# quokka-astro/quokka

Hardware: AMD Instinct MI355X
Metric: Mcell-updates/s on 3D Sedov unigrid (higher is better)
Workload: dtype f64; 1 GPU; 3D Sedov blast 256x256x256 unigrid (tests/blast_unigrid_256.in scaled to 256^3 cells per GPU), 128^3 boxes, PPM+HLLC RK2, gamma=1.4, CFL 0.3, reflecting octant; cells_per_gpu=16777216, boxes_per_gpu=8, parallelism=box-decomposition x1, rk2_mode=carry, fofc_stages=0, retries=0, x_sweep_in_y_march=True

## Files before the change

### include/quokka_amd.h

```cpp
#ifndef QUOKKA_AMD_H_
#define QUOKKA_AMD_H_

#include <stdint.h>

#ifdef __cplusplus
extern "C" {
#endif

typedef struct qk_ctx qk_ctx;
typedef struct qk_level qk_level;
typedef void *qk_stream;

typedef enum qk_status {
	QK_OK = 0,
	QK_ERR_INVALID = -1,
	QK_ERR_HIP = -2,
	QK_ERR_UNSUPPORTED = -3,
	QK_ERR_STATE = -4,
	QK_ERR_NOT_CONVERGED = -5
} qk_status;

typedef struct qk_array4 {
	double *p;
	int64_t jstride, kstride, nstride;
// ... 95 lines not shown
typedef struct qk_hydro_stage_args {
	const qk_array4 *U_in;
	const qk_array4 *U_old;
	qk_array4 *U_out;
	qk_array4 *halfFlux[3];
	qk_array4 *halfVel[3];
	qk_iarray4 *redoFlag;
	int64_t *d_redo_count;
	int *d_error_flag;
	double *d_max_signal;
	void *scratch;
	int64_t scratch_bytes;
	double dx[3];
	double dt;
	int stage;
	int reconstruction_order;
	double densityFloor, tempFloor;
	int use_dual_energy;
	double K_visc;
	int store_flux_rk2;
	qk_array4 *fluxRk2[3];
	int rk2_carry_rhs;
	qk_array4 *rhs1;
	const struct qk_carray4 *flux_mask;
	int fofc_pass;
	int prim_out;
	int prim_in;
	int store_vel_rk2;
	qk_array4 *velRk2[3];
} qk_hydro_stage_args;

int64_t qk_hydro_stage_scratch_bytes(qk_level *lev, const qk_hydro_traits *t);
int qk_hydro_stage_fused(qk_level *lev, qk_stream s, const qk_hydro_traits *t, const qk_hydro_stage_args *a);

#define QK_MAX_GROUPS 8
typedef struct qk_rad_traits {
	double c_light, c_hat, radiation_constant, Erad_floor;
	int beta_order;
	int opacity_model;
	double kappaP, kappaE, kappaF;
	int pow_mode;
	int eddington_model;
	double opacity_T_ref, opacity_T_exponent, opacity_pow_floor;
	int ngroups;
	int mg_opacity_model;
	double energy_unit;
	double rad_boundaries[QK_MAX_GROUPS + 1];
	double mg_kappa_exponent[QK_MAX_GROUPS + 1], mg_kappa_lower[QK_MAX_GROUPS + 1];
	double mg_kappa_rho_exponent, mg_kappa_T_ref, mg_kappa_T_exponent;
	int enable_dust_gas_thermal_coupling_model;
	double dust_gas_interaction_coeff;
	int thermal_model;
	double gas_dust_coupling_threshold;
	double cooling_linear_coeff[QK_MAX_GROUPS];
	double cr_heating_rate;
	int enable_photoelectric_heating;
	double pe_heating_E1_derivative;
} qk_rad_traits;

int qk_rad_ConservedToPrimitive(qk_level *lev, qk_stream s, const qk_rad_traits *rt, const qk_array4 *cons, qk_array4 *primVar, int nghost);
int qk_rad_ComputeWavespeedCorrection(qk_level *lev, qk_stream s, const qk_rad_traits *rt, const qk_hydro_traits *t, int ndim, const qk_array4 *consVar,
				      const double dx[3], qk_array4 *const eps[3]);
int qk_rad_ComputeFluxes(qk_level *lev, qk_stream s, const qk_rad_traits *rt, int dir, qk_array4 *x1Flux, const qk_array4 *x1LeftState,
			 const qk_array4 *x1RightState, const qk_array4 *consVar, const qk_array4 *wavespeed_eps);
int qk_rad_computeRadiationFluxes(qk_level *lev, qk_stream s, const qk_rad_traits *rt, int ndim, int reconstruction_order, const qk_array4 *consVar,
				  qk_array4 *const flux[3], const qk_array4 *const wavespeed_eps[3] );
// ... 200 lines not shown
```

### quokka_amd/capi.py

```python
from __future__ import annotations

import ctypes as C
import os

_HERE = os.path.dirname(os.path.abspath(__file__))
LIB_PATH = os.environ.get("QK_LIB_PATH", os.path.join(_HERE, "lib", "libquokka_amd.so"))

QK_OK, QK_ERR_INVALID, QK_ERR_HIP, QK_ERR_UNSUPPORTED, QK_ERR_STATE, QK_ERR_NOT_CONVERGED = 0, -1, -2, -3, -4, -5
ERR_UNSUPPORTED = QK_ERR_UNSUPPORTED
QK_TRACER_PREV, QK_TRACER_CUR, QK_TRACER_MAX_DEPTH = 0, 1, 3
HOOK_COMPILED = 100
DIR_X1, DIR_X2, DIR_X3 = 0, 1, 2
ARITH_DIVBY_RECIPOF, ARITH_DIVN, ARITH_RECIPEXACT, ARITH_SQRTN = 0, 1, 2, 3
COOLING_LIBM_DEVICE, COOLING_LIBM_PORTABLE = 0, 1
RIEMANN_HLLC, RIEMANN_LLF, RIEMANN_HLLD = 0, 1, 2
LIMITER_MINMOD, LIMITER_MC = 0, 1
BC_REFLECT_ODD, BC_INT_DIR, BC_REFLECT_EVEN, BC_FOEXTRAP, BC_EXT_DIR = -1, 0, 1, 2, 3

K_B = 1.380649e-16
M_U = 1.6605390666e-24


class Array4(C.Structure):
    _fields_ = [("p", C.c_void_p), ("jstride", C.c_int64), ("kstride", C.c_int64), ("nstride", C.c_int64),
# ... 118 lines not shown
    L.qk_ReconstructStatesConstant.argtypes = [vp, vp, ci, vp, vp, vp, ci, ci]
    L.qk_ReconstructStatesPLM.argtypes = [vp, vp, ci, ci, vp, vp, vp, ci, ci]
    L.qk_ReconstructStatesPPM.argtypes = [vp, vp, ci, vp, vp, vp, ci, ci, ci, ci]
    L.qk_hydro_ConservedToPrimitive.argtypes = [vp, vp, T, vp, vp, ci]
    L.qk_hydro_ComputeFlatteningCoefficients.argtypes = [vp, vp, T, ci, vp, vp, ci]
    L.qk_hydro_FlattenShocks.argtypes = [vp, vp, T, ci, vp, vp, vp, vp, vp, vp, ci, ci]
    L.qk_hydro_ComputeFluxes.argtypes = [vp, vp, T, ci, ci, vp, vp, vp, vp, vp, cd]
    L.qk_hydro_ComputeRhsFromFluxes.argtypes = [vp, vp, T, vp, P(vp), P(cd), ci]
    L.qk_hydro_AddInternalEnergyPdV.argtypes = [vp, vp, T, vp, vp, P(cd), P(vp), vp]
    L.qk_hydro_PredictStep.argtypes = [vp, vp, T, vp, vp, vp, cd, ci, vp, vp]
    L.qk_hydro_EnforceLimits.argtypes = [vp, vp, T, cd, cd, vp]
    L.qk_hydro_SyncDualEnergy.argtypes = [vp, vp, T, vp, vp]
    L.qk_hydro_ComputeMaxSignalSpeed.argtypes = [vp, vp, T, vp, vp]
    L.qk_hydro_maxSignalSpeedLocal.argtypes = [vp, vp, T, ci, vp, vp]
    L.qk_replaceFluxes.argtypes = [vp, vp, ci, vp, vp, vp, ci]
    L.qk_Saxpy.argtypes = [vp, vp, ci, vp, cd, vp, ci]
    R = P(RadTraits)
    L.qk_rad_ConservedToPrimitive.argtypes = [vp, vp, R, vp, vp, ci]
    L.qk_rad_ComputeFluxes.argtypes = [vp, vp, R, ci, vp, vp, vp, vp, vp]
    L.qk_rad_computeRadiationFluxes.argtypes = [vp, vp, R, ci, ci, vp, P(vp), P(vp)]
    L.qk_rad_ComputeWavespeedCorrection.argtypes = [vp, vp, R, T, ci, vp, P(cd), P(vp)]
    L.qk_rad_PredictStep.argtypes = [vp, vp, R, ci, vp, vp, P(vp), cd, P(cd)]
    L.qk_rad_AddFluxesRK2.argtypes = [vp, vp, R, ci, vp, vp, vp, P(vp), P(vp), cd, P(cd)]
    L.qk_hydro_FixupState.argtypes = [vp, vp, T, cd, cd, ci, vp, vp, vp]
    L.qk_rad_stage_fused.argtypes = [vp, vp, R, ci, ci, vp, vp, vp, vp, P(vp), cd, P(cd), P(vp)]
    L.qk_rad_AddSourceTermsSingleGroup.argtypes = [vp, vp, R, T, vp, vp, cd, ci, vp, vp]
    L.qk_rad_AddSourceTermsSingleGroupMirror.argtypes = [vp, vp, R, T, vp, vp, cd, ci, vp, vp, vp]
    L.qk_rad_AddSourceTermsMultiGroup.argtypes = [vp, vp, R, T, vp, vp, cd, ci, vp, vp]
    L.qk_rad_mg_planck_fractions.argtypes = [vp, R, cd, ci, P(cd), P(cd), P(cd)]
    if hasattr(L, "qk_hydro_stage_fused"):
        L.qk_hydro_stage_scratch_bytes.argtypes = [vp, T]
        L.qk_hydro_stage_scratch_bytes.restype = C.c_int64
        L.qk_hydro_stage_fused.argtypes = [vp, vp, T, P(StageArgs)]
    if hasattr(L, "qk_ghost_plan_create"):
        L.qk_ghost_plan_create.argtypes = [vp, P(vp), P(Geometry), ci, ci, ci, P(Box), P(ci), ci]
        L.qk_ghost_plan_destroy.argtypes = [vp]
        L.qk_ghost_plan_num_peers.argtypes = [vp]
        L.qk_ghost_plan_peer.argtypes = [vp, ci, P(ci), P(C.c_int64), P(C.c_int64)]
        L.qk_ghost_plan_num_items.argtypes = [vp, ci, ci]
        L.qk_ghost_plan_item.argtypes = [vp, ci, ci, ci, P(ci), P(ci), ci * 3, ci * 3, ci * 3, P(C.c_int64)]
        L.qk_FillBoundary_local.argtypes = [vp, vp, vp]
        L.qk_FillBoundary_local_int.argtypes = [vp, vp, vp]
        L.qk_FillBoundary_pack.argtypes = [vp, vp, ci, vp, vp]
        L.qk_FillBoundary_unpack.argtypes = [vp, vp, ci, vp, vp]
        L.qk_SumBoundary_local.argtypes = [vp, vp, vp]
        L.qk_SumBoundary_pack.argtypes = [vp, vp, ci, vp, vp]
        L.qk_SumBoundary_unpack.argtypes = [vp, vp, ci, vp, vp]
        L.qk_FillBoundary_pack_int.argtypes = [vp, vp, ci, vp, vp]
        L.qk_FillBoundary_unpack_int.argtypes = [vp, vp, ci, vp, vp]
        L.qk_FillPhysicalBoundary.argtypes = [vp, vp, vp, P(BCRec), P(DirichletFace)]
        L.qk_FillPhysicalBoundary_subset.argtypes = [vp, vp, vp, P(BCRec), P(DirichletFace), C.c_int]
        L.qk_ghost_plan_set_components.argtypes = [vp, C.c_int, C.c_int]
        L.qk_ghost_plan_box_is_remote.argtypes = [vp, C.c_int]
        L.qk_ghost_plan_set_box_remote.argtypes = [vp, C.c_int, C.c_int]
    if hasattr(L, "qk_tag_relative_gradient"):
        L.qk_tag_relative_gradient.argtypes = [vp, vp, T, vp, vp, ci, C.c_double, C.c_double, ci]
        L.qk_tag_centered_gradient.argtypes = [vp, vp, vp, vp, ci, ci, C.c_double, C.c_double, C.c_double, ci]
        L.qk_avgdown_plan_create.argtypes = [vp, vp, ci * 3, P(vp)]
        L.qk_avgdown_plan_destroy.argtypes = [vp]
        L.qk_avgdown_plan_num_items.argtypes = [vp]
        L.qk_average_down.argtypes = [vp, vp, vp, vp, ci, ci]
        L.qk_interp_plan_create.argtypes = [vp, vp, P(Geometry), ci, ci * 3, ci, ci, vp, P(vp)]
        L.qk_interp_plan_destroy.argtypes = [vp]
        L.qk_interp_plan_num_items.argtypes = [vp]
        L.qk_interp_plan_item.argtypes = [vp, ci, P(ci), P(ci), ci * 3, ci * 3]
        L.qk_InterpFromCoarse.argtypes = [vp, vp, vp, vp, vp, C.c_double, C.c_double, ci, ci, ci]
# ... 32 lines not shown
    L.qk_tracer_AdvectWithUmac.argtypes = [vp, vp, vp * 3, cd, C.c_int64, vp * 3, vp * 3]
    L.qk_tracer_Redistribute.argtypes = [vp, vp, C.c_int64, vp * 3, vp]
    L.qk_tracer_plan_create_refined.argtypes = [vp, P(vp), P(Geometry), cd * 3, cd * 3, cd * 3]
    L.qk_tracer_plan_set_parent.argtypes = [vp, ci, vp, vp * 3]
    L.qk_tracer_plan_set_time_weights.argtypes = [vp, cd, cd]
    L.qk_tracer_plan_clear_parent.argtypes = [vp]
    L.qk_tracer_Where.argtypes = [P(vp), ci, vp, ci, ci, C.c_int64, vp * 3, vp, vp, vp]
    i3 = ci * 3
    L.qk_gravity_scratch_bytes.argtypes = [i3]
    L.qk_gravity_scratch_bytes.restype = C.c_int64
    L.qk_gravity_num_ghosts.argtypes = [i3]
    L.qk_gravity_num_ghosts.restype = C.c_int64
    L.qk_gravity_fill_rhs.argtypes = [vp, vp, cd, vp, ci, i3, vp]
    L.qk_gravity_dirichlet_solve.argtypes = [vp, vp, i3, cd, vp, vp, cd, cd, ci, vp, C.c_int64, P(ci), P(cd)]
    L.qk_gravity_surface_gather.argtypes = [vp, vp, i3, vp, vp]
    L.qk_gravity_surface_potential.argtypes = [vp, vp, i3, vp, vp, vp, C.c_int64]
    L.qk_gravity_surface_scatter.argtypes = [vp, vp, i3, vp, vp]
    L.qk_gravity_kick.argtypes = [vp, vp, i3, vp, cd * 3, cd, vp]
    _lib = L
    return L


BOXES_ALL, BOXES_LOCAL_ONLY, BOXES_REMOTE_DEPENDENT = 0, 1, 2
TAG_CLEAR, TAG_BUF, TAG_SET = 0, 1, 2
TAGFIELD_PRESSURE = -1

DECLARED_SYMBOLS = [
    "qk_ctx_create", "qk_ctx_destroy", "qk_last_error", "qk_version", "qk_level_create", "qk_level_destroy",
    "qk_upload_array4_table", "qk_upload_iarray4_table", "qk_clear_bytes", "qk_profile_enable", "qk_profile_only", "qk_profile_reset", "qk_profile_num_kernels", "qk_profile_get",
    "qk_ReconstructStatesConstant", "qk_ReconstructStatesPLM", "qk_ReconstructStatesPPM",
    "qk_hydro_ConservedToPrimitive", "qk_hydro_ComputeFlatteningCoefficients", "qk_hydro_FlattenShocks",
    "qk_hydro_ComputeFluxes", "qk_hydro_ComputeRhsFromFluxes", "qk_hydro_AddInternalEnergyPdV", "qk_hydro_PredictStep",
    "qk_hydro_EnforceLimits", "qk_hydro_SyncDualEnergy", "qk_hydro_ComputeMaxSignalSpeed", "qk_hydro_maxSignalSpeedLocal",
    "qk_replaceFluxes", "qk_Saxpy", "qk_hydro_FixupState", "qk_hydro_stage_scratch_bytes", "qk_hydro_stage_fused",
    "qk_rad_ConservedToPrimitive", "qk_rad_ComputeWavespeedCorrection", "qk_rad_ComputeFluxes", "qk_rad_computeRadiationFluxes", "qk_rad_PredictStep", "qk_rad_AddFluxesRK2", "qk_rad_stage_fused",
    "qk_rad_AddSourceTermsSingleGroup", "qk_rad_AddSourceTermsSingleGroupMirror", "qk_rad_AddSourceTermsMultiGroup", "qk_rad_mg_planck_fractions",
    "qk_ghost_plan_create", "qk_ghost_plan_destroy", "qk_ghost_plan_num_peers", "qk_ghost_plan_peer", "qk_ghost_plan_num_items", "qk_ghost_plan_item",
    "qk_FillBoundary_local", "qk_FillBoundary_local_int", "qk_FillBoundary_pack", "qk_FillBoundary_unpack", "qk_FillBoundary_pack_int", "qk_FillBoundary_unpack_int", "qk_SumBoundary_local", "qk_SumBoundary_pack", "qk_SumBoundary_unpack", "qk_FillPhysicalBoundary",
    "qk_FillPhysicalBoundary_subset", "qk_ghost_plan_set_components", "qk_ghost_plan_box_is_remote", "qk_ghost_plan_set_box_remote",
    "qk_tag_relative_gradient", "qk_tag_centered_gradient", "qk_avgdown_plan_create", "qk_avgdown_plan_destroy", "qk_avgdown_plan_num_items", "qk_average_down", "qk_PreInterpState", "qk_PostInterpState",
    "qk_interp_plan_create", "qk_interp_plan_destroy", "qk_interp_plan_num_items", "qk_interp_plan_item", "qk_InterpFromCoarse",
    "qk_fluxreg_create", "qk_fluxreg_destroy", "qk_fluxreg_num_items", "qk_fluxreg_item", "qk_fluxreg_reset", "qk_fluxreg_save", "qk_fluxreg_restore", "qk_fluxreg_CrseAdd", "qk_fluxreg_FineAdd",
    "qk_fluxreg_Reflux", "qk_fluxreg_set_state_component", "qk_amr_tile_flags", "qk_amr_tile_flags_periodic", "qk_amr_cluster_tiles", "qk_amr_cluster_berger_rigoutsos", "qk_copy_box",
    "qk_cloudy_tables_read", "qk_cloudy_tables_free", "qk_cooling_tabulated", "qk_cooling_evaluate", "qk_cooling_set_libm", "qk_arith_evaluate",
    "qk_fluxreg_create_crse_part", "qk_pcopy_plan_create", "qk_pcopy_plan_destroy", "qk_pcopy_plan_num_peers", "qk_pcopy_plan_peer", "qk_pcopy_plan_num_items",
    "qk_pcopy_plan_item", "qk_ParallelCopy_local", "qk_ParallelCopy_pack", "qk_ParallelCopy_unpack",
    "qk_tracer_plan_create", "qk_tracer_plan_destroy", "qk_tracer_plan_lattice", "qk_tracer_InitOnePerCell", "qk_tracer_AdvectWithUmac", "qk_tracer_Redistribute",
    "qk_tracer_plan_create_refined", "qk_tracer_plan_set_parent", "qk_tracer_plan_set_time_weights", "qk_tracer_plan_clear_parent", "qk_tracer_Where",
    "qk_gravity_scratch_bytes", "qk_gravity_num_ghosts", "qk_gravity_fill_rhs", "qk_gravity_dirichlet_solve", "qk_gravity_surface_gather",
    "qk_gravity_surface_potential", "qk_gravity_surface_scatter", "qk_gravity_kick",
]


def check(ctx, rc: int, what: str = "") -> None:
    if rc != QK_OK:
        msg = lib().qk_last_error(ctx).decode() if ctx else ""
        raise QkError(f"{what} failed with status {rc}: {msg}")
```

### quokka_amd/csrc/qk_hydro_fused.hip

```cpp
#include "qk_device.hpp"
#include <algorithm>
#include <cmath>
#include <cstdlib>
#include <type_traits>
#include <vector>

#include "qk_internal.hpp"

using namespace qk;

namespace
{

constexpr int NG = 4;

template <class P> QK_DEV void streamStore(P *p, double v) { __builtin_nontemporal_store(v, p); }
template <class P> QK_DEV auto streamLoad(P *p) -> double { return __builtin_nontemporal_load(p); }

struct SGeom {
	int64_t off;
	int glo[3];
	int n[3];
	int pitch;
	int64_t ncell;
// ... 5 lines not shown

struct SweepArgs {
	const qk_box *boxes;
	const SGeom *geom;
	double *scratch;
	int64_t total_cells;
	const qk_array4 *U_in;
	const qk_array4 *U_old;
	qk_array4 *U_out;
	qk_array4 *halfFlux;
	qk_array4 *halfVel;
	qk_iarray4 *redoFlag;
	unsigned long long *redo_count;
	int *error_flag;
	double *max_signal;
	double inv_dx;
	double dx;
	double inv_dx0, dx0;
	double dx3[3];
	double dt;
	double densityFloor, tempFloor;
	double K_visc;
	int use_dual_energy;
	bool reconstruct_eint;
	bool same_old;
	bool store_rk2;
	qk_array4 *rk2Flux;
	qk_array4 *rhs1;
	const qk_carray4 *fluxMask;
	int nseg;
	bool prim_in, prim_out;
	bool store_vel;
	qk_array4 *rk2Vel;
};

QK_DEV auto sarr(SweepArgs const &a, int comp) -> double * { return a.scratch + static_cast<int64_t>(comp) * a.total_cells; }

#ifndef QK_PT_Y
#define QK_PT_Y 7
#define QK_PT_THREADS 512
#endif
constexpr int PT_X = 66, PT_Y = QK_PT_Y, PT_THREADS = QK_PT_THREADS;
constexpr int PT_OWN = PT_X * PT_Y;
constexpr int PT_HALO_Y = 6 * PT_X;
constexpr int PT_HALO = PT_HALO_Y + 6 * PT_Y;
static_assert(PT_HALO <= PT_THREADS && PT_OWN <= PT_THREADS, "one halo cell per thread");

struct PlaneCell {
	double rho, vx, vy, vz, P;
};

struct PlaneRaw {
	double rho, mx, my, mz, E;
};
QK_DEV auto planeLoad(RA4 const &U, int64_t u) -> PlaneRaw
{
	PlaneRaw r;
	r.rho = U.p[u + U.ns * RHO];
	r.mx = U.p[u + U.ns * MX];
	r.my = U.p[u + U.ns * MY];
	r.mz = U.p[u + U.ns * MZ];
	r.E = U.p[u + U.ns * ENE];
	return r;
}
QK_DEV auto planeCell(Eos const &eos, bool re, PlaneRaw const &r) -> PlaneCell
{
// ... 766 lines not shown
	const int mrow = min(row0 + brow, hi);
	const int f = x0 + 64 * side;
	int64_t ub = Uin.idx(f - 3, mrow, ot);
	double qb[6][NV], Uc[NVAR];
#pragma unroll
	for (int m = 0; m < 6; ++m, ++ub) {
		loadPrims<NS>(Uin, ub, eos, a.reconstruct_eint, a.prim_in, qb[m], Uc);
	}
	const int64_t cb = (f - 1 - g.glo[0]) + (mrow - g.glo[1]) * st[1] + (ot - g.glo[2]) * st[2];
	const double chiL = S[cb], chiR = S[cb + 1];
	const double DyL = S[(S_AUX + 2) * T + cb], DyR = S[(S_AUX + 2) * T + cb + 1];
	const double DzL = S[(S_AUX + 3) * T + cb], DzR = S[(S_AUX + 3) * T + cb + 1];
	double qLb[NV], qRb[NV], Fb[NV], vfb;
#pragma unroll
	for (int n = 0; n < NV; ++n) {
		double unused;
		reconstructVar<ORDER>(chiL, qb[0][n], qb[1][n], qb[2][n], qb[3][n], qb[4][n], unused, qLb[n]);
		reconstructVar<ORDER>(chiR, qb[1][n], qb[2][n], qb[3][n], qb[4][n], qb[5][n], qRb[n], unused);
	}
	faceFluxAll<0, QK_RIEMANN_HLLC, false, NS>(eos, a.reconstruct_eint, 3, qLb, qRb, qb[3][PVX] - qb[2][PVX], DyL, DyR, DzL, DzR, a.K_visc, Fb, vfb);
	double(*ed)[NV + 1] = edge[brow];
	double *ef = ed[5 - side];
#pragma unroll
	for (int n = 0; n < NV; ++n) {
		ef[n] = Fb[n];
	}
	ef[NV] = vfb;
#pragma unroll
	for (int n = 0; n < NV; ++n) {
		ed[2 * side][n] = (side != 0) ? qb[3][n] : qb[1][n];
		ed[2 * side + 1][n] = (side != 0) ? qb[4][n] : qb[2][n];
	}
}
template <int DIR, int ORDER, int STAGE, bool LAST, int NS, bool CARRY, bool TWOD = false, bool FOFC = false, bool FUSEX = false>
__global__ void __launch_bounds__(64 * MARCH_BY) k_sweep_march(SweepArgs a, Eos eos)
{
	static_assert(!FUSEX || (DIR == 1 && !LAST && !TWOD && !FOFC && CARRY), "the X sweep rides on the Y sweep of a 3-D level in the carried form");
	static_assert(!(FOFC && CARRY), "the first-order flux correction pass exists for the reference's form of the RK2 average");
	static_assert(!TWOD || (DIR == 1 && LAST), "the 2-D build has one marching sweep: y, carrying the epilogue");
	constexpr int NV = NVAR + NS;
	constexpr int RHS_DIVV = S_RHS + NV;
	static_assert(DIR == 1 || DIR == 2, "marching sweeps are the strided directions");
	const BlockId blk = xcdContiguousBlock();
	const int bix = blk.x, biy = blk.y, biz = blk.z;
	const int b = biz / a.nseg;
	const int seg = biz - b * a.nseg;
	const qk_box bx = a.boxes[b];
	const SGeom g = a.geom[b];
	constexpr int OT = (DIR == 1) ? 2 : 1;
	const int i_raw = bx.lo[0] + bix * 64 + threadIdx.x;
	const int ot_raw = bx.lo[OT] + biy * MARCH_BY + threadIdx.y;
	const bool live = (i_raw <= bx.hi[0]) && (ot_raw <= bx.hi[OT]);
	const int i = min(i_raw, bx.hi[0]);
	const int ot = min(ot_raw, bx.hi[OT]);
	double sig0 = 0., sig1 = 0.;
	const int64_t T = a.total_cells;
	const int64_t st[3] = {1, g.pitch, static_cast<int64_t>(g.pitch) * g.n[1]};
	const int64_t ms = st[DIR];
	const int seglen = (bx.hi[DIR] - bx.lo[DIR] + 1 + a.nseg - 1) / a.nseg;
	const int lo = bx.lo[DIR] + seg * seglen, hi = min(lo + seglen - 1, bx.hi[DIR]);
	const int nvalid = hi - lo + 1;
	if (nvalid <= 0) {
		return;
	}
	if constexpr (FUSEX) {
		if (bx.lo[0] + bix * 64 > bx.hi[0]) {
			return;
		}
	}
	int pos[3];
	pos[0] = i;
	pos[OT] = ot;
	pos[DIR] = lo - 3;
	int64_t c = (pos[0] - g.glo[0]) * st[0] + (pos[1] - g.glo[1]) * st[1] + (pos[2] - g.glo[2]) * st[2];
	const double *S = a.scratch + g.off;
	double *Sw = a.scratch + g.off;
	RA4 Uin(a.U_in[b]);
	RA4 Uold(a.U_old[b]);
	const EpiConst ec = epiConst(eos);
	int64_t u = Uin.idx(pos[0], pos[1], pos[2]);
	const int64_t ums = (DIR == 1) ? Uin.js : Uin.ks;

	constexpr int AV = Axes<DIR, TWOD>::v, AW = Axes<DIR, TWOD>::w;
	double q[5][NV];
	double apPrev[NV], Fprev[NV];
	double vfPrev = 0., dVprev = 0., dWprev = 0.;
	bool maskCol = false;
	int maskLo = 0, maskHi = -1;
	if (CARRY && a.fluxMask != nullptr) {
		const qk_carray4 md = a.fluxMask[b];
		maskCol = live && i >= md.begin[0] && i < md.end[0] && ot >= md.begin[OT] && ot < md.end[OT];
		maskLo = md.begin[DIR];
		maskHi = md.end[DIR] - 1;
	}
	constexpr bool RING = LAST && (STAGE == 1);
	__shared__ double s_ring[RING ? 3 : 1][RING ? NV : 1][RING ? 64 * MARCH_BY : 1];
	__shared__ double s_fx[FUSEX ? MARCH_BY : 1][FUSEX ? NV + 2 : 1][FUSEX ? XW : 1];
	__shared__ double s_edge[FUSEX ? MARCH_BY : 1][FUSEX ? XROWS : 1][6][FUSEX ? NV + 1 : 1];
	double chiPrev = 1.;
	const int lself = (FUSEX && threadIdx.x == 0) ? 69 : static_cast<int>(threadIdx.x) + 2;
	const int lnext = (FUSEX && threadIdx.x == 63) ? 68 : static_cast<int>(threadIdx.x) + 3;
	const int tid = threadIdx.y * 64 + threadIdx.x;
	const bool ring = RING && a.same_old;
	int slot = 0;
	double Uo[NV];
#pragma unroll
	for (int n = 0; n < NV; ++n) {
		apPrev[n] = 0.;
		Fprev[n] = 0.;
#pragma unroll
		for (int m = 0; m < 5; ++m) {
			q[m][n] = 0.;
		}
	}

	constexpr bool PFQ = !FUSEX && NS == 0;
	double Un[NVAR];
	if constexpr (PFQ) {
#pragma unroll
		for (int n = 0; n < NVAR; ++n) {
			Un[n] = Uin.p[u + Uin.ns * n];
		}
	}
	for (int step = 0; step < nvalid + 6; ++step, c += ms, u += ums) {
#pragma unroll
		for (int n = 0; n < NV; ++n) {
			q[0][n] = q[1][n];
			q[1][n] = q[2][n];
			q[2][n] = q[3][n];
			q[3][n] = q[4][n];
		}
		{
			double Uc[NVAR];
			if constexpr (PFQ) {
#pragma unroll
				for (int n = 0; n < NVAR; ++n) {
					Uc[n] = Un[n];
					Un[n] = Uin.p[u + ums + Uin.ns * n];
				}
				primsOf<NS>(Uin, u, eos, a.reconstruct_eint, a.prim_in, Uc, q[4]);
			} else {
				loadPrims<NS>(Uin, u, eos, a.reconstruct_eint, a.prim_in, q[4], Uc);
// ... 57 lines not shown
				for (int n = 0; n < NV; ++n) {
					rhs_in[n] = a.inv_dx0 * (sx[n][lself] - sx[n][lnext]);
				}
				rhs_in[NV] = (sx[NV][lnext] - sx[NV][lself]) / a.dx0;
				waveFence();
				if (rr + 1 < XROWS) {
					stageEdgeRow<NV>(sx, edge[rr + 1]);
				}
			} else {
#pragma unroll
				for (int n = 0; n < NV + 1; ++n) {
					rhs_in[n] = streamLoad(&S[(S_RHS + n) * T + cu]);
				}
			}
			if (LAST && !ring && !(CARRY && STAGE == 2)) {
				const int64_t co = Uold.idx(cidx[0], cidx[1], cidx[2]);
#pragma unroll
				for (int n = 0; n < NV; ++n) {
					Uo[n] = Uold.p[co + Uold.ns * n];
				}
			}
			if (CARRY && LAST && STAGE == 2) {
				RA4 R1(a.rhs1[b]);
				const int64_t c1 = R1.idx(cidx[0], cidx[1], cidx[2]);
#pragma unroll
				for (int n = 0; n < NV + 1; ++n) {
					F1[n] = R1.p[c1 + R1.ns * n];
				}
			}
		}
		if (!CARRY && STAGE == 2 && step >= 5) {
			loadF1<NV>(a, b, fidx, F1);
		}
		double am[NV], ap[NV];
		reconstructCell<ORDER>(chi, q[2], [&](int m, int n) { return q[2 + m][n]; }, am, ap);
		if (step >= 5) {
			const double du = q[2][PVX + DIR] - q[1][PVX + DIR];
			double F[NV], vf;
			faceFluxAll<DIR, QK_RIEMANN_HLLC, TWOD, NS>(eos, a.reconstruct_eint, TWOD ? 2 : 3, apPrev, am, du, dVprev, dV, dWprev, dW, a.K_visc, F, vf);
			bool marked = false;
			if (maskCol && fidx[DIR] >= maskLo && cidx[DIR] <= maskHi) {
				CA4 M(a.fluxMask[b]);
				const int m0 = (cidx[DIR] >= maskLo) ? M(cidx[0], cidx[1], cidx[2]) : 0;
				const int m1 = (fidx[DIR] <= maskHi) ? M(fidx[0], fidx[1], fidx[2]) : 0;
				marked = (m0 | m1) != 0;
			}
			settleFace<STAGE, CARRY, FOFC, DIR, NS, TWOD>(a, eos, TWOD ? 2 : 3, b, fidx, live, marked, F1, q[1], q[2], F, vf);
			if (step >= 6) {
				double rhs[NV];
#pragma unroll
				for (int n = 0; n < NV; ++n) {
					rhs[n] = rhs_in[n] + a.inv_dx * (Fprev[n] - F[n]);
				}
				const double div_v = rhs_in[NV] + (vf - vfPrev) / a.dx;
				if (LAST) {
					if (live) {
						updateCellFrom<NS, CARRY ? STAGE : 0, FOFC, TWOD ? 2 : 3>(a, eos, ec, b, cidx[0], cidx[1], cidx[2], Uo, rhs, div_v, F1, sig0, sig1,
													    (STAGE == 1) && a.same_old && !a.reconstruct_eint && !a.prim_in, q[1][PPRES]);
					}
				} else if (live) {
#pragma unroll
					for (int n = 0; n < NV; ++n) {
						streamStore(&Sw[(S_RHS + n) * T + cu], rhs[n]);
					}
					streamStore(&Sw[RHS_DIVV * T + cu], div_v);
				}
			}
#pragma unroll
			for (int n = 0; n < NV; ++n) {
				Fprev[n] = F[n];
			}
			vfPrev = vf;
		}
#pragma unroll
		for (int n = 0; n < NV; ++n) {
			apPrev[n] = ap[n];
		}
		dVprev = dV;
		dWprev = dW;
		chiPrev = chi;
	}
	if (LAST && a.max_signal != nullptr) {
		reduceSignal(a.max_signal, sig0, sig1);
	}
}

inline auto smallLevelCells() -> int64_t
{
	static const int64_t v = [] {
		const char *e = std::getenv("QK_SMALL_LEVEL_CELLS");
		return (e != nullptr) ? static_cast<int64_t>(std::atoll(e)) : static_cast<int64_t>(2) << 20;
	}();
	return v;
}

inline auto smallMinLen() -> int
{
	static const int v = [] {
		const char *e = std::getenv("QK_SMALL_MINLEN");
		return (e != nullptr) ? std::max(1, std::atoi(e)) : 4;
	}();
	return v;
}

auto marchSegments(const qk_level *lev, int dir, int ot) -> int
{
	if (const char *e = std::getenv("QK_MARCH_SEGMENTS")) {
		return std::max(1, std::atoi(e));
	}
	const int64_t cols = static_cast<int64_t>(lev->nboxes) * lev->maxlen[0] * lev->maxlen[ot];
	const int64_t want = (131072 + cols - 1) / std::max<int64_t>(cols, 1);
	const int minlen = (cols * lev->maxlen[dir] < smallLevelCells()) ? smallMinLen() : 16;
	const int cap = std::max(1, lev->maxlen[dir] / minlen);
	return static_cast<int>(std::min<int64_t>(std::max<int64_t>(want, 1), std::min(cap, 16)));
}

// ... 64 lines not shown
			const double cost = (std::ceil(rounds) / rounds) * (static_cast<double>(seglen + 6) / seglen);
			if (cost < best) {
				best = cost;
				nseg = c;
			}
		}
	}
	return nseg;
}

auto sweepArgsFor(SweepArgs a, const qk_hydro_stage_args *args, int d) -> SweepArgs
{
	a.halfFlux = args->halfFlux[d];
	a.halfVel = args->halfVel[d];
	a.rk2Flux = args->fluxRk2[d];
	a.rk2Vel = args->velRk2[d];
	a.inv_dx = 1.0 / args->dx[d];
	a.dx = args->dx[d];
	return a;
}

auto fusexApplies(const qk_level *lev, SweepArgs const &a, bool carry, int nscalars) -> bool
{
	const char *e = std::getenv("QK_FUSEX");
	if (!carry || nscalars != 0 || lev->ndim != 3 || a.fluxMask != nullptr || (e != nullptr && std::atoi(e) == 0)) {
		return false;
	}
	for (int b = 0; b < lev->nboxes; ++b) {
		if ((lev->boxes[b].hi[0] - lev->boxes[b].lo[0] + 1) % 64 != 0) {
			return false;
		}
	}
	return true;
}

template <int ORDER, int STAGE, int NS, bool CARRY, bool FOFC = false> void launchSweeps(qk_level *lev, hipStream_t s, SweepArgs a, Eos eos, const qk_hydro_stage_args *args)
{
	const bool fusex = fusexApplies(lev, a, CARRY, NS);
	if (!fusex) {
		const SweepArgs ax = sweepArgsFor(a, args, 0);
		const int64_t slab = static_cast<int64_t>(lev->maxlen[0] + 2 * NG) * lev->maxlen[1];
		const dim3 grid(static_cast<unsigned>((slab + XOUT - 1) / XOUT), static_cast<unsigned>(lev->maxlen[2]), static_cast<unsigned>(lev->nboxes));
		ProfScope ps(lev->ctx, s, "k_sweep_x");
		if (lev->ndim == 3) {
			hipLaunchKernelGGL((k_sweep_x<ORDER, STAGE, NS, CARRY, 3, FOFC>), grid, dim3(XB), 0, s, ax, eos);
		} else if constexpr (!CARRY) {
			if (lev->ndim == 2) {
				hipLaunchKernelGGL((k_sweep_x<ORDER, STAGE, NS, false, 2, FOFC>), grid, dim3(XB), 0, s, ax, eos);
			} else {
				hipLaunchKernelGGL((k_sweep_x<ORDER, STAGE, NS, false, 1, FOFC>), grid, dim3(XB), 0, s, ax, eos);
			}
		}
	}
	if (lev->ndim == 1) {
		return;
	}
	{
		SweepArgs ay = sweepArgsFor(a, args, 1);
		ay.same_old = (lev->ndim == 2) && (args->U_in == args->U_old);
		ay.nseg = marchSegments(lev, 1, 2);
		ay.inv_dx0 = 1.0 / args->dx[0];
		ay.dx0 = args->dx[0];
		const dim3 grid((lev->maxlen[0] + 63) / 64, (lev->maxlen[2] + MARCH_BY - 1) / MARCH_BY, lev->nboxes * ay.nseg);
		ProfScope ps(lev->ctx, s, fusex ? "k_sweep_xy" : "k_sweep_y");
		if (lev->ndim == 2) {
			if constexpr (!CARRY) {
// ... 33 lines not shown
		}
	};
	if (args->stage == 1) {
		form(std::integral_constant<int, 1>{});
	} else {
		form(std::integral_constant<int, 2>{});
	}
}
template <int ORDER> void launchOrder(int nscalars, qk_level *lev, hipStream_t s, SweepArgs const &a, Eos const &eos, const qk_hydro_stage_args *args)
{
	switch (nscalars) {
	case 0: return launchStage<ORDER, 0>(lev, s, a, eos, args);
	case 1: return launchStage<ORDER, 1>(lev, s, a, eos, args);
	case 2: return launchStage<ORDER, 2>(lev, s, a, eos, args);
	default: return launchStage<ORDER, 3>(lev, s, a, eos, args);
	}
}

}

extern "C" {

int64_t qk_hydro_stage_scratch_bytes(qk_level *lev, const qk_hydro_traits *t)
{
	if (lev == nullptr) {
		return QK_ERR_INVALID;
	}
	if (int rc = checkTraits(lev->ctx, t); rc != QK_OK) {
		return rc;
	}
	std::vector<SGeom> g;
	const int64_t cells = scratchGeom(lev, g);
	return cells * scratchComps(t->nscalars) * static_cast<int64_t>(sizeof(double));
}

int qk_hydro_stage_fused(qk_level *lev, qk_stream stream, const qk_hydro_traits *t, const qk_hydro_stage_args *args)
{
	if (lev == nullptr) {
		return QK_ERR_INVALID;
	}
	qk_ctx *ctx = lev->ctx;
	if (int rc = checkTraits(ctx, t); rc != QK_OK) {
		return rc;
	}
	if (int rc = needsLibraryEos(ctx, t, "qk_hydro_stage_fused (EnforceLimits)"); rc != QK_OK) {
		return rc;
	}
	QK_REQUIRE(ctx, args != nullptr, "qk_hydro_stage_fused: NULL args");
	if (lev->nboxes == 0) {
		return QK_OK;
	}
	if (t->nscalars > QK_FUSED_MAX_SCALARS || t->nmscalars != 0) {
		return setError(ctx, QK_ERR_UNSUPPORTED, "qk_hydro_stage_fused: up to 3 passive scalars, no mass scalars (use the reference-shaped operators)");
	}
	if (t->ndim != lev->ndim) {
		return setError(ctx, QK_ERR_INVALID, "qk_hydro_stage_fused: traits.ndim differs from the level's dimension");
	}
	if (t->ndim != 3 && args->rk2_carry_rhs != 0) {
		return setError(ctx, QK_ERR_UNSUPPORTED, "qk_hydro_stage_fused: rk2_carry_rhs is instantiated for 3-D builds");
	}
	QK_REQUIRE(ctx, args->K_visc >= 0.0, "qk_hydro_stage_fused: negative artificial-viscosity coefficient");
	QK_REQUIRE(ctx, args->stage == 1 || args->stage == 2, "qk_hydro_stage_fused: stage must be 1 or 2");
	QK_REQUIRE(ctx, args->reconstruction_order >= 1 && args->reconstruction_order <= 3, "qk_hydro_stage_fused: reconstruction_order must be 1..3");
	QK_REQUIRE(ctx, args->U_in && args->U_old && args->U_out && args->redoFlag && args->d_redo_count && args->d_error_flag && args->scratch,
		   "qk_hydro_stage_fused: NULL array");
	QK_REQUIRE(ctx, args->fofc_pass == 0 || (args->K_visc == 0.0 && (args->rk2_carry_rhs == 0 || args->stage == 1)),
// ... 47 lines not shown
		const int nseg = prePassSegments(lev, xt, yt);
		const dim3 grid(static_cast<unsigned>(xt) * yt * lev->nboxes * nseg);
		if (args->prim_in != 0) {
			hipLaunchKernelGGL(k_pre3<true>, grid, dim3(PT_THREADS), 0, s, boxes, geom, args->U_in, scratch, T, eos, re, nseg, xt, yt, t->ndim);
		} else {
			hipLaunchKernelGGL(k_pre3<false>, grid, dim3(PT_THREADS), 0, s, boxes, geom, args->U_in, scratch, T, eos, re, nseg, xt, yt, t->ndim);
		}
	}

	SweepArgs a{};
	a.boxes = boxes;
	a.geom = geom;
	a.scratch = scratch;
	a.total_cells = T;
	a.U_in = args->U_in;
	a.U_old = args->U_old;
	a.U_out = args->U_out;
	a.redoFlag = args->redoFlag;
	a.redo_count = reinterpret_cast<unsigned long long *>(args->d_redo_count);
	a.error_flag = args->d_error_flag;
	a.max_signal = args->d_max_signal;
	a.dt = args->dt;
	a.densityFloor = args->densityFloor;
	a.tempFloor = args->tempFloor;
	a.K_visc = args->K_visc;
	a.use_dual_energy = args->use_dual_energy;
	a.reconstruct_eint = re;
	a.store_rk2 = (args->store_flux_rk2 != 0);
	a.store_vel = (args->store_vel_rk2 != 0);
	a.rhs1 = args->rhs1;
	a.fluxMask = (args->rk2_carry_rhs != 0) ? args->flux_mask : nullptr;
	a.prim_in = (args->prim_in != 0);
	a.prim_out = (args->prim_out != 0);
	for (int d = 0; d < 3; ++d) {
		a.dx3[d] = args->dx[d];
	}

	if (args->reconstruction_order == 3) {
		launchOrder<3>(t->nscalars, lev, s, a, eos, args);
	} else if (args->reconstruction_order == 2) {
		launchOrder<2>(t->nscalars, lev, s, a, eos, args);
	} else {
		launchOrder<1>(t->nscalars, lev, s, a, eos, args);
	}
	QK_HIP_CHECK(ctx, hipGetLastError());
	return QK_OK;
}

}
```

### quokka_amd/csrc/qk_internal.hpp

```cpp
#ifndef QK_INTERNAL_HPP_
#define QK_INTERNAL_HPP_

#include <hip/hip_runtime.h>

#include <cstdio>
#include <mutex>
#include <string>
#include <vector>

#include "quokka_amd.h"

struct qk_prof_pending {
	int slot;
	hipEvent_t start, stop;
};
struct qk_prof_slot {
	std::string name;
	long count = 0;
	double total_ms = 0.0;
};

struct qk_ctx {
	int device = 0;
	std::string last_error;
	std::vector<void *> owned;
	std::mutex mtx;
	bool profiling = false;
	std::string prof_only;
	std::vector<qk_prof_slot> prof_slots;
	std::vector<qk_prof_pending> prof_pending;
	std::vector<hipEvent_t> prof_free_events;
	int *counter_slots = nullptr;
	int cooling_libm = 0;
};

struct qk_level {
	qk_ctx *ctx = nullptr;
	int ndim = 3;
	int nboxes = 0;
	std::vector<qk_box> boxes;
	qk_box *d_boxes = nullptr;
	int maxlen[3] = {0, 0, 0};
	void *d_sgeom = nullptr;
	int64_t sgeom_total_cells = 0;
	int *d_tile_flags = nullptr;
	size_t tile_flags_bytes = 0;
	unsigned long long *d_cooling_queue = nullptr;
};

namespace qk
{

inline auto setError(qk_ctx *ctx, int code, const char *what, const char *detail = "") -> int
{
	if (ctx != nullptr) {
		std::lock_guard<std::mutex> lock(ctx->mtx);
		ctx->last_error = std::string(what) + (detail[0] != 0 ? ": " : "") + detail;
	}
	return code;
}

#define QK_HIP_CHECK(ctx, expr)                                                                                                                      \
	do {                                                                                                                                         \
		hipError_t qk_e_ = (expr);                                                                                                           \
		if (qk_e_ != hipSuccess) {                                                                                                           \
			return qk::setError((ctx), QK_ERR_HIP, #expr, hipGetErrorString(qk_e_));                                                     \
		}                                                                                                                                    \
	} while (0)

#define QK_REQUIRE(ctx, cond, msg)                                                                                                                   \
	do {                                                                                                                                         \
		if (!(cond)) {                                                                                                                       \
			return qk::setError((ctx), QK_ERR_INVALID, msg);                                                                             \
		}                                                                                                                                    \
	} while (0)

inline auto checkTraits(qk_ctx *ctx, const qk_hydro_traits *t) -> int
{
	if (t == nullptr) {
		return setError(ctx, QK_ERR_INVALID, "traits is NULL");
// ... 94 lines not shown
```

Before: 3196 Mcell-updates/s.

## Reuse face fluxes across wave-uniform runs in the marching hydro sweep

In the marching sweep kernel, each step now checks with wave-wide ballots whether the incoming cells and transverse coefficients are bitwise identical to the previous ones. After a long enough uniform run, it reuses the previous face flux (and reconstruction) instead of redoing PPM reconstruction and the HLLC solve. An adaptive back-off limits how often the checks run, and a device counter can record skipped steps. This targets the large quiescent ambient region of problems like Sedov. In exchange it adds ballot and compare overhead, extra registers, and a launch-bounds minimum of two blocks per CU for the affected instantiations, which may cause spills. It is on by default and can be turned off with an environment variable.

New measurement: 3517 Mcell-updates/s, median of 6. 10.1% higher.

```diff
diff --git a/include/quokka_amd.h b/include/quokka_amd.h
--- a/include/quokka_amd.h
+++ b/include/quokka_amd.h
@@ -151,6 +151,7 @@
 
 int64_t qk_hydro_stage_scratch_bytes(qk_level *lev, const qk_hydro_traits *t);
 int qk_hydro_stage_fused(qk_level *lev, qk_stream s, const qk_hydro_traits *t, const qk_hydro_stage_args *a);
+int qk_hydro_stage_set_skip_counter(qk_level *lev, void *d_count);
 
 #define QK_MAX_GROUPS 8
 typedef struct qk_rad_traits {
diff --git a/quokka_amd/capi.py b/quokka_amd/capi.py
--- a/quokka_amd/capi.py
+++ b/quokka_amd/capi.py
@@ -174,6 +174,8 @@
         L.qk_hydro_stage_scratch_bytes.argtypes = [vp, T]
         L.qk_hydro_stage_scratch_bytes.restype = C.c_int64
         L.qk_hydro_stage_fused.argtypes = [vp, vp, T, P(StageArgs)]
+        if hasattr(L, "qk_hydro_stage_set_skip_counter"):
+            L.qk_hydro_stage_set_skip_counter.argtypes = [vp, vp]
     if hasattr(L, "qk_ghost_plan_create"):
         L.qk_ghost_plan_create.argtypes = [vp, P(vp), P(Geometry), ci, ci, ci, P(Box), P(ci), ci]
         L.qk_ghost_plan_destroy.argtypes = [vp]
@@ -272,7 +274,7 @@
     "qk_hydro_ConservedToPrimitive", "qk_hydro_ComputeFlatteningCoefficients", "qk_hydro_FlattenShocks",
     "qk_hydro_ComputeFluxes", "qk_hydro_ComputeRhsFromFluxes", "qk_hydro_AddInternalEnergyPdV", "qk_hydro_PredictStep",
     "qk_hydro_EnforceLimits", "qk_hydro_SyncDualEnergy", "qk_hydro_ComputeMaxSignalSpeed", "qk_hydro_maxSignalSpeedLocal",
-    "qk_replaceFluxes", "qk_Saxpy", "qk_hydro_FixupState", "qk_hydro_stage_scratch_bytes", "qk_hydro_stage_fused",
+    "qk_replaceFluxes", "qk_Saxpy", "qk_hydro_FixupState", "qk_hydro_stage_scratch_bytes", "qk_hydro_stage_fused", "qk_hydro_stage_set_skip_counter",
     "qk_rad_ConservedToPrimitive", "qk_rad_ComputeWavespeedCorrection", "qk_rad_ComputeFluxes", "qk_rad_computeRadiationFluxes", "qk_rad_PredictStep", "qk_rad_AddFluxesRK2", "qk_rad_stage_fused",
     "qk_rad_AddSourceTermsSingleGroup", "qk_rad_AddSourceTermsSingleGroupMirror", "qk_rad_AddSourceTermsMultiGroup", "qk_rad_mg_planck_fractions",
     "qk_ghost_plan_create", "qk_ghost_plan_destroy", "qk_ghost_plan_num_peers", "qk_ghost_plan_peer", "qk_ghost_plan_num_items", "qk_ghost_plan_item",
diff --git a/quokka_amd/csrc/qk_hydro_fused.hip b/quokka_amd/csrc/qk_hydro_fused.hip
--- a/quokka_amd/csrc/qk_hydro_fused.hip
+++ b/quokka_amd/csrc/qk_hydro_fused.hip
@@ -61,6 +61,8 @@
 	bool prim_in, prim_out;
 	bool store_vel;
 	qk_array4 *rk2Vel;
+	bool uniform_skip;
+	unsigned long long *skip_count;
 };
 
 QK_DEV auto sarr(SweepArgs const &a, int comp) -> double * { return a.scratch + static_cast<int64_t>(comp) * a.total_cells; }
@@ -893,9 +895,22 @@
 		ed[2 * side + 1][n] = (side != 0) ? qb[4][n] : qb[2][n];
 	}
 }
+QK_DEV auto sameBits(double x, double y) -> bool { return __double_as_longlong(x) == __double_as_longlong(y); }
+QK_DEV auto waveAll(bool v) -> bool { return __ballot(v) == ~0ull; }
+template <int NV> QK_DEV auto sameCell(const double (&x)[NV], const double (&y)[NV]) -> bool
+{
+	bool same = true;
+#pragma unroll
+	for (int n = 0; n < NV; ++n) {
+		same = same & sameBits(x[n], y[n]);
+	}
+	return same;
+}
+constexpr auto marchRepeats(int NS, bool TWOD, int STAGE) -> bool { return NS == 0 || (NS == 1 && !(TWOD && STAGE == 2)); }
 template <int DIR, int ORDER, int STAGE, bool LAST, int NS, bool CARRY, bool TWOD = false, bool FOFC = false, bool FUSEX = false>
-__global__ void __launch_bounds__(64 * MARCH_BY) k_sweep_march(SweepArgs a, Eos eos)
-{
+__global__ void __launch_bounds__(64 * MARCH_BY, marchRepeats(NS, TWOD, STAGE) ? 2 : 1) k_sweep_march(SweepArgs a, Eos eos)
+{
+	constexpr bool USKIP = marchRepeats(NS, TWOD, STAGE);
 	static_assert(!FUSEX || (DIR == 1 && !LAST && !TWOD && !FOFC && CARRY), "the X sweep rides on the Y sweep of a 3-D level in the carried form");
 	static_assert(!(FOFC && CARRY), "the first-order flux correction pass exists for the reference's form of the RK2 average");
 	static_assert(!TWOD || (DIR == 1 && LAST), "the 2-D build has one marching sweep: y, carrying the epilogue");
@@ -946,6 +961,9 @@
 	double q[5][NV];
 	double apPrev[NV], Fprev[NV];
 	double vfPrev = 0., dVprev = 0., dWprev = 0.;
+	constexpr bool RAWF = USKIP && !CARRY && (STAGE == 2 || FOFC);
+	int runCells = 0, runCoef = 0, nRepeat = 0, idle = 0, pause = 1;
+	double Fraw[RAWF ? NV : 1], vfRaw = 0.;
 	bool maskCol = false;
 	int maskLo = 0, maskHi = -1;
 	if (CARRY && a.fluxMask != nullptr) {
@@ -969,6 +987,9 @@
 	for (int n = 0; n < NV; ++n) {
 		apPrev[n] = 0.;
 		Fprev[n] = 0.;
+		if constexpr (RAWF) {
+			Fraw[n] = 0.;
+		}
 #pragma unroll
 		for (int m = 0; m < 5; ++m) {
 			q[m][n] = 0.;
@@ -1092,49 +1113,161 @@
 		if (!CARRY && STAGE == 2 && step >= 5) {
 			loadF1<NV>(a, b, fidx, F1);
 		}
-		double am[NV], ap[NV];
-		reconstructCell<ORDER>(chi, q[2], [&](int m, int n) { return q[2 + m][n]; }, am, ap);
-		if (step >= 5) {
-			const double du = q[2][PVX + DIR] - q[1][PVX + DIR];
-			double F[NV], vf;
-			faceFluxAll<DIR, QK_RIEMANN_HLLC, TWOD, NS>(eos, a.reconstruct_eint, TWOD ? 2 : 3, apPrev, am, du, dVprev, dV, dWprev, dW, a.K_visc, F, vf);
-			bool marked = false;
-			if (maskCol && fidx[DIR] >= maskLo && cidx[DIR] <= maskHi) {
-				CA4 M(a.fluxMask[b]);
-				const int m0 = (cidx[DIR] >= maskLo) ? M(cidx[0], cidx[1], cidx[2]) : 0;
-				const int m1 = (fidx[DIR] <= maskHi) ? M(fidx[0], fidx[1], fidx[2]) : 0;
-				marked = (m0 | m1) != 0;
-			}
-			settleFace<STAGE, CARRY, FOFC, DIR, NS, TWOD>(a, eos, TWOD ? 2 : 3, b, fidx, live, marked, F1, q[1], q[2], F, vf);
-			if (step >= 6) {
-				double rhs[NV];
+		bool repeat = false;
+		if (USKIP && a.uniform_skip) {
+			if (idle > 0) {
+				--idle;
+				runCells = 0;
+				runCoef = 0;
+			} else {
+				const bool allC = waveAll(sameCell<NV>(q[4], q[3]));
+				const bool allK = waveAll(sameBits(chi, chiPrev) & sameBits(dV, dVprev) & sameBits(dW, dWprev));
+				runCells = allC ? runCells + 1 : 0;
+				runCoef = (allK && step > 4) ? runCoef + 1 : 0;
+				if (allC && (allK || step == 4)) {
+					pause = 1;
+				} else {
+					idle = pause;
+					pause = min(2 * pause, 8);
+				}
+				repeat = runCells >= 6 && runCoef >= 2;
+				nRepeat += repeat ? 1 : 0;
+			}
+		}
+		if constexpr (!USKIP) {
+			double am[NV], ap[NV];
+			reconstructCell<ORDER>(chi, q[2], [&](int m, int n) { return q[2 + m][n]; }, am, ap);
+			if (step >= 5) {
+				const double du = q[2][PVX + DIR] - q[1][PVX + DIR];
+				double F[NV], vf;
+				faceFluxAll<DIR, QK_RIEMANN_HLLC, TWOD, NS>(eos, a.reconstruct_eint, TWOD ? 2 : 3, apPrev, am, du, dVprev, dV, dWprev, dW, a.K_visc, F, vf);
+				bool marked = false;
+				if (maskCol && fidx[DIR] >= maskLo && cidx[DIR] <= maskHi) {
+					CA4 M(a.fluxMask[b]);
+					const int m0 = (cidx[DIR] >= maskLo) ? M(cidx[0], cidx[1], cidx[2]) : 0;
+					const int m1 = (fidx[DIR] <= maskHi) ? M(fidx[0], fidx[1], fidx[2]) : 0;
+					marked = (m0 | m1) != 0;
+				}
+				settleFace<STAGE, CARRY, FOFC, DIR, NS, TWOD>(a, eos, TWOD ? 2 : 3, b, fidx, live, marked, F1, q[1], q[2], F, vf);
+				if (step >= 6) {
+					double rhs[NV];
+#pragma unroll
+					for (int n = 0; n < NV; ++n) {
+						rhs[n] = rhs_in[n] + a.inv_dx * (Fprev[n] - F[n]);
+					}
+					const double div_v = rhs_in[NV] + (vf - vfPrev) / a.dx;
+					if (LAST) {
+						if (live) {
+							updateCellFrom<NS, CARRY ? STAGE : 0, FOFC, TWOD ? 2 : 3>(a, eos, ec, b, cidx[0], cidx[1], cidx[2], Uo, rhs, div_v, F1, sig0, sig1,
+														    (STAGE == 1) && a.same_old && !a.reconstruct_eint && !a.prim_in, q[1][PPRES]);
+						}
+					} else if (live) {
+#pragma unroll
+						for (int n = 0; n < NV; ++n) {
+							streamStore(&Sw[(S_RHS + n) * T + cu], rhs[n]);
+						}
+						streamStore(&Sw[RHS_DIVV * T + cu], div_v);
+					}
+				}
 #pragma unroll
 				for (int n = 0; n < NV; ++n) {
-					rhs[n] = rhs_in[n] + a.inv_dx * (Fprev[n] - F[n]);
-				}
-				const double div_v = rhs_in[NV] + (vf - vfPrev) / a.dx;
-				if (LAST) {
-					if (live) {
-						updateCellFrom<NS, CARRY ? STAGE : 0, FOFC, TWOD ? 2 : 3>(a, eos, ec, b, cidx[0], cidx[1], cidx[2], Uo, rhs, div_v, F1, sig0, sig1,
-													    (STAGE == 1) && a.same_old && !a.reconstruct_eint && !a.prim_in, q[1][PPRES]);
+					Fprev[n] = F[n];
+				}
+				vfPrev = vf;
+			}
+#pragma unroll
+			for (int n = 0; n < NV; ++n) {
+				apPrev[n] = ap[n];
+			}
+		} else {
+			constexpr bool SPLIT = CARRY && NS == 0;
+			auto finishFace = [&](double (&F)[NV], double &vf) {
+				if constexpr (RAWF) {
+#pragma unroll
+					for (int n = 0; n < NV; ++n) {
+						Fraw[n] = F[n];
 					}
-				} else if (live) {
+					vfRaw = vf;
+				}
+				bool marked = false;
+				if (maskCol && fidx[DIR] >= maskLo && cidx[DIR] <= maskHi) {
+					CA4 M(a.fluxMask[b]);
+					const int m0 = (cidx[DIR] >= maskLo) ? M(cidx[0], cidx[1], cidx[2]) : 0;
+					const int m1 = (fidx[DIR] <= maskHi) ? M(fidx[0], fidx[1], fidx[2]) : 0;
+					marked = (m0 | m1) != 0;
+				}
+				settleFace<STAGE, CARRY, FOFC, DIR, NS, TWOD>(a, eos, TWOD ? 2 : 3, b, fidx, live, marked, F1, q[1], q[2], F, vf);
+				if (step >= 6) {
+					double rhs[NV];
 #pragma unroll
 					for (int n = 0; n < NV; ++n) {
-						streamStore(&Sw[(S_RHS + n) * T + cu], rhs[n]);
+						rhs[n] = rhs_in[n] + a.inv_dx * (Fprev[n] - F[n]);
 					}
-					streamStore(&Sw[RHS_DIVV * T + cu], div_v);
-				}
-			}
-#pragma unroll
-			for (int n = 0; n < NV; ++n) {
-				Fprev[n] = F[n];
-			}
-			vfPrev = vf;
-		}
-#pragma unroll
-		for (int n = 0; n < NV; ++n) {
-			apPrev[n] = ap[n];
+					const double div_v = rhs_in[NV] + (vf - vfPrev) / a.dx;
+					if (LAST) {
+						if (live) {
+							updateCellFrom<NS, CARRY ? STAGE : 0, FOFC, TWOD ? 2 : 3>(a, eos, ec, b, cidx[0], cidx[1], cidx[2], Uo, rhs, div_v, F1, sig0, sig1,
+														    (STAGE == 1) && a.same_old && !a.reconstruct_eint && !a.prim_in, q[1][PPRES]);
+						}
+					} else if (live) {
+#pragma unroll
+						for (int n = 0; n < NV; ++n) {
+							streamStore(&Sw[(S_RHS + n) * T + cu], rhs[n]);
+						}
+						streamStore(&Sw[RHS_DIVV * T + cu], div_v);
+					}
+				}
+#pragma unroll
+				for (int n = 0; n < NV; ++n) {
+					Fprev[n] = F[n];
+				}
+				vfPrev = vf;
+			};
+			if (SPLIT && repeat && !FUSEX) {
+				double F[NV], vf;
+#pragma unroll
+				for (int n = 0; n < NV; ++n) {
+					if constexpr (RAWF) {
+						F[n] = Fraw[n];
+					} else {
+						F[n] = Fprev[n];
+					}
+				}
+				vf = RAWF ? vfRaw : vfPrev;
+				finishFace(F, vf);
+			} else {
+				double am[NV], ap[NV];
+				if (!SPLIT && repeat) {
+#pragma unroll
+					for (int n = 0; n < NV; ++n) {
+						ap[n] = apPrev[n];
+					}
+				} else {
+					reconstructCell<ORDER>(chi, q[2], [&](int m, int n) { return q[2 + m][n]; }, am, ap);
+				}
+				if (step >= 5) {
+					double F[NV], vf;
+					if (repeat) {
+#pragma unroll
+						for (int n = 0; n < NV; ++n) {
+							if constexpr (RAWF) {
+								F[n] = Fraw[n];
+							} else {
+								F[n] = Fprev[n];
+							}
+						}
+						vf = RAWF ? vfRaw : vfPrev;
+					} else {
+						const double du = q[2][PVX + DIR] - q[1][PVX + DIR];
+						faceFluxAll<DIR, QK_RIEMANN_HLLC, TWOD, NS>(eos, a.reconstruct_eint, TWOD ? 2 : 3, apPrev, am, du, dVprev, dV, dWprev, dW, a.K_visc, F, vf);
+					}
+					finishFace(F, vf);
+				}
+#pragma unroll
+				for (int n = 0; n < NV; ++n) {
+					apPrev[n] = ap[n];
+				}
+			}
 		}
 		dVprev = dV;
 		dWprev = dW;
@@ -1142,6 +1275,11 @@
 	}
 	if (LAST && a.max_signal != nullptr) {
 		reduceSignal(a.max_signal, sig0, sig1);
+	}
+	if constexpr (USKIP) {
+		if (a.skip_count != nullptr && threadIdx.x == 0 && live && nRepeat > 0) {
+			atomicAdd(&a.skip_count[0], static_cast<unsigned long long>(nRepeat));
+		}
 	}
 }
 
@@ -1272,6 +1410,12 @@
 		}
 	}
 	return true;
+}
+
+auto uniformSkipOn() -> bool
+{
+	const char *e = std::getenv("QK_UNIFORM_SKIP");
+	return e == nullptr || std::atoi(e) != 0;
 }
 
 template <int ORDER, int STAGE, int NS, bool CARRY, bool FOFC = false> void launchSweeps(qk_level *lev, hipStream_t s, SweepArgs a, Eos eos, const qk_hydro_stage_args *args)
@@ -1371,6 +1515,15 @@
 	std::vector<SGeom> g;
 	const int64_t cells = scratchGeom(lev, g);
 	return cells * scratchComps(t->nscalars) * static_cast<int64_t>(sizeof(double));
+}
+
+int qk_hydro_stage_set_skip_counter(qk_level *lev, void *d_count)
+{
+	if (lev == nullptr) {
+		return QK_ERR_INVALID;
+	}
+	lev->d_skip_count = static_cast<unsigned long long *>(d_count);
+	return QK_OK;
 }
 
 int qk_hydro_stage_fused(qk_level *lev, qk_stream stream, const qk_hydro_traits *t, const qk_hydro_stage_args *args)
@@ -1484,6 +1637,8 @@
 	a.fluxMask = (args->rk2_carry_rhs != 0) ? args->flux_mask : nullptr;
 	a.prim_in = (args->prim_in != 0);
 	a.prim_out = (args->prim_out != 0);
+	a.uniform_skip = uniformSkipOn();
+	a.skip_count = lev->d_skip_count;
 	for (int d = 0; d < 3; ++d) {
 		a.dx3[d] = args->dx[d];
 	}
diff --git a/quokka_amd/csrc/qk_internal.hpp b/quokka_amd/csrc/qk_internal.hpp
--- a/quokka_amd/csrc/qk_internal.hpp
+++ b/quokka_amd/csrc/qk_internal.hpp
@@ -46,6 +46,7 @@
 	int *d_tile_flags = nullptr;
 	size_t tile_flags_bytes = 0;
 	unsigned long long *d_cooling_queue = nullptr;
+	unsigned long long *d_skip_count = nullptr;
 };
 
 namespace qk
```
